# yflyzhang/RankPO

Hardware: AMD Instinct MI355X
Metric: query-passage pairs/sec (higher is better)
Workload: dtype bf16

## Files before the change

### include/rankpo_hip.h

```cpp
#ifndef RANKPO_HIP_H
#define RANKPO_HIP_H

#include <stddef.h>
#include <stdint.h>

#ifdef __cplusplus
extern "C" {
#endif

typedef void* rpo_stream_t;

typedef enum {
    RPO_OK = 0,
    RPO_ERR_INVALID_ARG = -1,
    RPO_ERR_UNSUPPORTED = -2,
    RPO_ERR_WORKSPACE = -3,
    RPO_ERR_LAUNCH = -4
} rpo_status;

typedef enum { RPO_DT_F32 = 0, RPO_DT_BF16 = 1, RPO_DT_F16 = 2 } rpo_dtype;
typedef enum { RPO_POOL_LAST = 0, RPO_POOL_CLS = 1 } rpo_pool_mode;
typedef enum { RPO_TARGET_INBATCH = 0, RPO_TARGET_FIRST = 1 } rpo_target_mode;
typedef enum { RPO_LOSS_SIGMOID = 0, RPO_LOSS_HINGE = 1 } rpo_loss_type;

// ... 86 lines not shown
                          int dtype, float lr, float beta1, float beta2, float eps, float weight_decay, const void* ls_state,
                          rpo_stream_t stream);

int rpo_swiglu_fwd(const void* g, const void* u, void* out, int64_t rows, int64_t cols, int64_t ld_gu, int64_t ld_out,
                   int dtype, rpo_stream_t stream);
int rpo_swiglu_bwd(const void* g, const void* u, const void* dout, void* dg, void* du, void* prod_out, int64_t rows,
                   int64_t cols, int64_t ld_gu, int64_t ld_dout, int64_t ld_dgu, int64_t ld_prod, int dtype,
                   rpo_stream_t stream);
int rpo_swiglu_bwd_t(const void* g, const void* u, const void* dout, void* dg, void* du, void* prod_t_out, void* dgu_t_out,
                     int64_t rows, int64_t cols, int64_t ld_gu, int64_t ld_dout, int64_t ld_dgu, int64_t ld_t, int dtype,
                     rpo_stream_t stream);
int rpo_rope(const void* x_in, void* x_out, int64_t row_stride, const float* cos_tab, const float* sin_tab,
             int64_t rows, int64_t heads, int64_t head_dim, int64_t period, int dtype, int backward,
             rpo_stream_t stream);

int rpo_transpose(const void* in, void* out, int64_t rows, int64_t cols, int64_t ld_in, int64_t ld_out, int dtype,
                  rpo_stream_t stream);

int rpo_add_rmsnorm_waves(int64_t rows);
int rpo_add_rmsnorm_fwd(const void* x, const void* delta, const void* weight, float eps, void* x_out, void* y_out,
                        float* rstd_out, int64_t rows, int64_t d, int dtype, rpo_stream_t stream);
int rpo_add_rmsnorm_bwd(const void* dy, const void* x_new, const void* weight, const float* rstd, const void* dres,
                        void* dx_out, float* dw_partial, int64_t rows, int64_t d, int dtype, rpo_stream_t stream);

int rpo_flash_attn_fwd(const void* q, const void* k, const void* v, int64_t q_stride, int64_t k_stride,
                       int64_t v_stride, const int* cu_seqlens, const int* tiles, int64_t ntiles, int64_t tile_cols,
                       int64_t total_tokens,
                       int64_t num_heads, int64_t num_kv_heads, int64_t head_dim, float scale, void* out,
                       int64_t out_stride, float* lse, int64_t lse_max_len, const float* rope_cos, const float* rope_sin,
                       int64_t rope_period, int64_t q_block, rpo_stream_t stream);

int rpo_flash_attn_bwd(const void* q, const void* k, const void* v, const void* out, const void* dout, int64_t q_stride,
                       int64_t k_stride, int64_t v_stride, int64_t out_stride, int64_t dout_stride,
                       const int* cu_seqlens, const int* q_tiles, int64_t n_q_tiles, int64_t q_tile_cols, const int* k_tiles,
                       int64_t n_k_tiles, int64_t key_block, int64_t sweep_down, int64_t total_tokens, int64_t num_heads,
                       int64_t num_kv_heads, int64_t head_dim, float scale, const float* lse, float* delta, void* dq, void* dk, void* dv,
                       int64_t dq_stride, int64_t dk_stride, int64_t dv_stride, const float* rope_cos, const float* rope_sin,
                       int64_t rope_period, int64_t q_block, rpo_stream_t stream);

int rpo_lastq_attn_fwd(const void* q, int64_t q_stride, const void* k, const void* v, int64_t k_stride, int64_t v_stride,
                       const int* cu_seqlens, int64_t num_seqs, int64_t num_heads, int64_t num_kv_heads, int64_t head_dim,
                       float scale, void* out, int64_t out_stride, float* lse, rpo_stream_t stream);
int rpo_lastq_attn_bwd(const void* q, int64_t q_stride, const void* k, const void* v, int64_t k_stride, int64_t v_stride,
                       const int* cu_seqlens, int64_t num_seqs, int64_t num_heads, int64_t num_kv_heads, int64_t head_dim,
                       float scale, const void* out, int64_t out_stride, const void* dout, int64_t dout_stride, const float* lse,
                       void* dq, int64_t dq_stride, void* dk, void* dv, int64_t dk_stride, int64_t dv_stride, rpo_stream_t stream);
// ... 104 lines not shown
```

### rankpo_amd/_lib.py

```python
from __future__ import annotations

import ctypes as C
import os

_HERE = os.path.dirname(os.path.abspath(__file__))
LIB_PATH = os.path.join(_HERE, "csrc", "librankpo_hip.so")

RPO_OK = 0
RPO_DT_F32, RPO_DT_BF16, RPO_DT_F16 = 0, 1, 2
RPO_POOL_LAST, RPO_POOL_CLS = 0, 1
(RPO_LS_SCALE, RPO_LS_MULT, RPO_LS_NORM, RPO_LS_SKIP, RPO_LS_GOOD_STEPS, RPO_LS_CUR_HYSTERESIS, RPO_LS_APPLIED_STEPS,
 RPO_LS_SKIPPED_STEPS, RPO_LS_FLOOR_HITS) = range(9)
RPO_LS_WORDS = 16
RPO_TARGET_INBATCH, RPO_TARGET_FIRST = 0, 1
RPO_LOSS_SIGMOID, RPO_LOSS_HINGE = 0, 1
RPO_BUILD_ONEWAVE64 = 1
RPO_NUM_METRICS = 9
METRIC_KEYS = (
    "rankpo_loss", "sft_loss", "rewards/chosen", "rewards/rejected", "rewards/accuracies",
    "rewards/margins", "scores/chosen", "scores/rejected", "scores/margins",
)


class RankPOParams(C.Structure):
# ... 27 lines not shown
    "rpo_rankpo_fwd": (C.c_int, [_vp, _vp, _vp, _vp, _i64, _i64, _i32, C.POINTER(RankPOParams), _vp, _vp, _vp, _vp, _vp, _vp]),
    "rpo_rankpo_bwd": (C.c_int, [_vp, _vp, _vp, _vp, _i64, _i64, _i32, _vp, _vp, _vp]),
    "rpo_adamw_step": (C.c_int, [_vp, _vp, _vp, _vp, _vp, _i64, _i32, _f32, _f32, _f32, _f32, _f32, _f32, _f32, _vp, _vp]),
    "rpo_sumsq_partial": (C.c_int, [_vp, _i64, _i32, _vp, _i32, _vp]),
    "rpo_loss_scale_update": (C.c_int, [_vp, _vp, _f32, _f32, _i32, _i32, _i32, _i32, _f32, _vp]),
    "rpo_adamw_step_scaled": (C.c_int, [_vp, _vp, _vp, _vp, _vp, _i64, _i32, _f32, _f32, _f32, _f32, _f32, _vp, _vp]),
    "rpo_swiglu_fwd": (C.c_int, [_vp, _vp, _vp, _i64, _i64, _i64, _i64, _i32, _vp]),
    "rpo_topk_merge": (C.c_int, [_vp, _i64, _i64, _i64, _i64, _i32, _i32, _vp, _vp, _i32, _vp]),
    "rpo_topk_merge_split": (C.c_int, [_vp, _i64, _i64, _i64, _i64, _i32, _i32, _i32, _vp, _vp, _i32, _vp]),
    "rpo_sim_topk_filter_ok": (C.c_int, [_i64, _i64, _i64]),
    "rpo_sim_topk_filter": (C.c_int, [_vp, _vp, _i64, _i64, _i64, _i32, _i64, _i32, _i32, _vp, _vp, _vp, _vp, _vp, _i32, _vp]),
    "rpo_sim_scores_f32": (C.c_int, [_vp, _vp, _i64, _i64, _i64, _i32, _vp, _i64, _vp]),
    "rpo_topk_merge_candidates": (C.c_int, [_vp, _vp, _vp, _i64, _i32, _i32, _vp, _vp, _vp, _vp]),
    "rpo_split_bf16x3": (C.c_int, [_vp, _i64, _i64, _i64, _vp, _i64, _vp, _vp]),
    "rpo_sim_planes_ok": (C.c_int, [_i64, _i64, _i64]),
    "rpo_sim_scores_f32_planes": (C.c_int, [_vp, _vp, _i64, _i64, _i64, _vp, _i64, _vp]),
    "rpo_sim_topk_filter_planes": (C.c_int, [_vp, _vp, _i64, _i64, _i64, _i64, _i32, _vp, _vp, _vp, _vp, _vp, _i32, _vp]),
    "rpo_swiglu_bwd": (C.c_int, [_vp, _vp, _vp, _vp, _vp, _vp, _i64, _i64, _i64, _i64, _i64, _i64, _i32, _vp]),
    "rpo_swiglu_bwd_t": (C.c_int, [_vp, _vp, _vp, _vp, _vp, _vp, _vp, _i64, _i64, _i64, _i64, _i64, _i64, _i32, _vp]),
    "rpo_transpose": (C.c_int, [_vp, _vp, _i64, _i64, _i64, _i64, _i32, _vp]),
    "rpo_add_rmsnorm_waves": (C.c_int, [_i64]),
    "rpo_add_rmsnorm_fwd": (C.c_int, [_vp, _vp, _vp, _f32, _vp, _vp, _vp, _i64, _i64, _i32, _vp]),
    "rpo_add_rmsnorm_bwd": (C.c_int, [_vp, _vp, _vp, _vp, _vp, _vp, _vp, _i64, _i64, _i32, _vp]),
    "rpo_flash_attn_fwd": (C.c_int, [_vp, _vp, _vp, _i64, _i64, _i64, _vp, _vp, _i64, _i64, _i64, _i64, _i64, _i64, _f32, _vp,
                                     _i64, _vp, _i64, _vp, _vp, _i64, _i64, _vp]),
    "rpo_flash_attn_bwd": (C.c_int, [_vp] * 5 + [_i64] * 5 + [_vp, _vp, _i64, _i64, _vp, _i64, _i64, _i64, _i64, _i64, _i64, _i64, _f32, _vp, _vp,
                                     _vp, _vp, _vp, _i64, _i64, _i64, _vp, _vp, _i64, _i64, _vp]),
    "rpo_lastq_attn_fwd": (C.c_int, [_vp, _i64, _vp, _vp, _i64, _i64, _vp, _i64, _i64, _i64, _i64, _f32, _vp, _i64, _vp, _vp]),
    "rpo_lastq_attn_bwd": (C.c_int, [_vp, _i64, _vp, _vp, _i64, _i64, _vp, _i64, _i64, _i64, _i64, _f32, _vp, _i64, _vp, _i64, _vp,
                                     _vp, _i64, _vp, _vp, _i64, _i64, _vp]),
    "rpo_rope": (C.c_int, [_vp, _vp, _i64, _vp, _vp, _i64, _i64, _i64, _i64, _i32, _i32, _vp]),
    "rpo_bidir_attn_fwd": (C.c_int, [_vp, _vp, _vp, _i64, _i64, _i64, _vp, _vp, _vp, _i64, _i64, _i64, _i64, _i64, _i64, _i64, _i32,
                                     _f32, _vp, _i64, _vp, _vp]),
    "rpo_add_layernorm_fwd": (C.c_int, [_vp, _i64, _vp, _i64, _vp, _vp, _f32, _vp, _i64, _i64, _i64, _i32, _vp]),
    "rpo_gelu_fwd": (C.c_int, [_vp, _i64, _i64, _i64, _i32, _vp]),
    "rpo_bert_embed_ln_fwd": (C.c_int, [_vp, _vp, _vp, _i64, _vp, _i64, _vp, _i64, _vp, _i64, _vp, _vp, _f32, _vp, _i64, _i64, _i32,
                                        _vp]),
    "rpo_bidir_attn_fwd_f32": (C.c_int, [_vp, _vp, _vp, _i64, _i64, _i64, _vp, _vp, _vp, _i64, _i64, _i64, _i64, _i64, _i64, _i64,
                                         _f32, _vp, _i64, _vp, _vp]),
    "rpo_add_layernorm_fwd_f32": (C.c_int, [_vp, _i64, _vp, _i64, _vp, _vp, _f32, _vp, _i64, _i64, _i64, _vp]),
    "rpo_gelu_fwd_f32": (C.c_int, [_vp, _i64, _i64, _i64, _vp]),
    "rpo_bert_embed_ln_fwd_f32": (C.c_int, [_vp, _vp, _vp, _i64, _vp, _i64, _vp, _i64, _vp, _i64, _vp, _vp, _f32, _vp, _i64, _i64,
                                            _vp]),
    "rpo_bidir_attn_train_fwd": (C.c_int, [_vp, _vp, _vp, _i64, _i64, _i64, _vp, _vp, _vp, _i64, _i64, _i64, _i64, _i64, _i64, _i64,
                                           _i32, _f32, _f32, _u64, _vp, _i64, _vp, _vp]),
    "rpo_bidir_attn_bwd": (C.c_int, [_vp, _vp, _vp, _i64, _i64, _i64, _vp, _i64, _vp, _i64, _vp, _vp, _vp, _vp, _i64, _vp, _i64,
# ... 55 lines not shown
```

### rankpo_amd/csrc/encoder_ops.hip

```cpp
#include "common.hpp"

namespace {

constexpr int kEwThreads = 256;

__device__ __forceinline__ float sigmoid_f(float x) { return 1.0f / (1.0f + __expf(-x)); }

template <typename T>
__global__ __launch_bounds__(kEwThreads) void swiglu_fwd_kernel(const T* __restrict__ g, const T* __restrict__ u,
                                                                T* __restrict__ out, int64_t rows, int vec_per_row,
                                                                int64_t ld_gu, int64_t ld_out) {
    constexpr int V = Elem<T>::kVec;
    const int64_t i = (int64_t)blockIdx.x * kEwThreads + threadIdx.x;
    const int64_t r = i / vec_per_row;
    if (r >= rows) return;
    const int c = (int)(i - r * vec_per_row) * V;
    Vec16<T> a, b, o;
    a.load_nt(g + r * ld_gu + c);
    b.load_nt(u + r * ld_gu + c);
#pragma unroll
    for (int k = 0; k < V; ++k) o.v[k] = a.v[k] * sigmoid_f(a.v[k]) * b.v[k];
    o.store_nt(out + r * ld_out + c);
}

// ... 551 lines not shown
        (delta && (!rpo_aligned16(delta) || !rpo_aligned16(x_out))))
        return RPO_ERR_UNSUPPORTED;
    hipStream_t st = (hipStream_t)stream;
    const int nw = norm_waves(rows, RPO_NORM_FWD_CAP);
    if (dtype == RPO_DT_BF16) return launch_norm_fwd<bf16_t>(x, delta, weight, eps, x_out, y_out, rstd_out, rows, d, nw, st);
    if (dtype == RPO_DT_F32) return launch_norm_fwd<float>(x, delta, weight, eps, x_out, y_out, rstd_out, rows, d, nw, st);
    return RPO_ERR_INVALID_ARG;
}

extern "C" int rpo_add_rmsnorm_bwd(const void* dy, const void* x_new, const void* weight, const float* rstd,
                                   const void* dres, void* dx_out, float* dw_partial, int64_t rows, int64_t d,
                                   int dtype, rpo_stream_t stream) {
    if (!dy || !x_new || !weight || !rstd || !dx_out || !dw_partial || rows <= 0 || d <= 0) return RPO_ERR_INVALID_ARG;
    const int V = dtype == RPO_DT_BF16 ? 8 : 4;
    if (d % V != 0 || !rpo_aligned16(dy) || !rpo_aligned16(x_new) || !rpo_aligned16(dx_out) || !rpo_aligned16(weight) ||
        !rpo_aligned16(dw_partial) || (dres && !rpo_aligned16(dres)))
        return RPO_ERR_UNSUPPORTED;
    hipStream_t st = (hipStream_t)stream;
    const int nw = rpo_add_rmsnorm_waves(rows);
    if (dtype == RPO_DT_BF16) return launch_norm_bwd<bf16_t>(dy, x_new, weight, rstd, dres, dx_out, dw_partial, rows, d, nw, st);
    if (dtype == RPO_DT_F32) return launch_norm_bwd<float>(dy, x_new, weight, rstd, dres, dx_out, dw_partial, rows, d, nw, st);
    return RPO_ERR_INVALID_ARG;
}
```

### rankpo_amd/distributed.py

```python
from __future__ import annotations

from typing import List, Optional

import torch
import torch.distributed as dist


def _all_gather_into(out: torch.Tensor, x: torch.Tensor, async_op=False):
    if dist.get_backend() == "nccl":
        return dist.all_gather_into_tensor(out.view(-1), x.reshape(-1), async_op=async_op)
    if x.is_cuda:
        host = [torch.empty(x.shape, dtype=x.dtype) for _ in range(out.shape[0])]
        dist.all_gather(host, x.cpu())
        out.copy_(torch.stack(host).to(out.device))
        return None
    return dist.all_gather(list(out.unbind(0)), x, async_op=async_op)


def deal_balanced(costs, hands: int) -> List[List[int]]:
    n = len(costs)
    if hands <= 0 or n % hands:
        raise ValueError(f"cannot deal {n} items into {hands} equal hands")
    per = n // hands
    total = [0.0] * hands
# ... 113 lines not shown

    def wait(self) -> torch.Tensor:
        if self.work is not None:
            self.work.wait()
            self.work = None
        return self.out.view((-1,) + tuple(self.x.shape[1:]))


class FusedQPGather:

    def __init__(self, qp: torch.Tensor, num_queries: int):
        self.nq = int(num_queries)
        self._g = EmbeddingGather(qp)

    def wait(self):
        out = self._g.out
        self._g.wait()
        d = out.shape[-1]
        return out[:, :self.nq].reshape(-1, d), out[:, self.nq:].reshape(-1, d)


def gather_embeddings(q: torch.Tensor, p: torch.Tensor):
    return FusedQPGather(torch.cat([q.detach(), p.detach()], 0), q.shape[0]).wait()


class FlatGradAllReducer:

    def __init__(self, params: List[torch.nn.Parameter], bucket_mb: float = 512.0, world_size: Optional[int] = None,
                 force_collectives: bool = False, shard: bool = False, rank: Optional[int] = None):
        self.params = [p for p in params if p.requires_grad]
        self.world = world_size if world_size is not None else (dist.get_world_size() if dist.is_initialized() else 1)
        self.rank = rank if rank is not None else (dist.get_rank() if dist.is_initialized() else 0)
        self.shard = bool(shard)
        assert self.params, "no trainable parameters"
        dtype, device = self.params[0].dtype, self.params[0].device
        assert all(p.dtype == dtype and p.device == device for p in self.params), "one dtype/device per reducer"
        order = list(reversed(self.params))
        i = 0
        while i < len(order):
            tag = getattr(order[i], "_rpo_fuse_group", None)
            j = i + 1
            if tag is not None:
                while j < len(order) and getattr(order[j], "_rpo_fuse_group", (None,))[0] is tag[0]:
                    j += 1
                order[i:j] = sorted(order[i:j], key=lambda p: p._rpo_fuse_group[1])
            i = j
# ... 7 lines not shown
            offs.append(n)
            n += (p.numel() + 7) // 8 * 8
            idxs.append(i)
            if n - start >= per or i == len(order) - 1:
                n = start + (n - start + quantum - 1) // quantum * quantum
                self.buckets.append((start, n, idxs))
                start, idxs = n, []
        self.numel = n
        self.flat = torch.zeros(n, dtype=dtype, device=device)
        self.order, self.offsets = order, offs
        for p, o in zip(order, offs):
            p.grad = self.flat[o:o + p.numel()].view_as(p)
        self.shard_offsets, self.shard_numel, self.grad_shards = [], 0, None
        if self.shard:
            for s_, e_, _ in self.buckets:
                self.shard_offsets.append(self.shard_numel)
                self.shard_numel += (e_ - s_) // self.world
            self.grad_shards = torch.zeros(self.shard_numel, dtype=dtype, device=device)
        self._bucket_of = {}
        for b, (_, _, ids) in enumerate(self.buckets):
            for i in ids:
                self._bucket_of[i] = b
        self._pending = [0] * len(self.buckets)
        self._works = []
        self._armed = False
        self.late_buckets = 0
        self._reduce = self.world > 1 or (force_collectives and dist.is_initialized())
        if self._reduce:
            for i, p in enumerate(order):
                p.register_post_accumulate_grad_hook(self._make_hook(i))

    def _make_hook(self, i):
        def hook(param):
            o = self.offsets[i]
            view = self.flat[o:o + param.numel()].view_as(param)
            if param.grad is not None and param.grad.data_ptr() != view.data_ptr():
                view.copy_(param.grad)
                param.grad = view
            if not self._armed:
                return
            b = self._bucket_of[i]
            self._pending[b] -= 1
            if self._pending[b] == 0:
                self._works.append(self._reduce_bucket(b))
        return hook

    def shard_view(self, b: int) -> torch.Tensor:
        s, e, _ = self.buckets[b]
        o = self.shard_offsets[b]
        return self.grad_shards[o:o + (e - s) // self.world]

    def _reduce_bucket(self, b: int):
        s, e, _ = self.buckets[b]
        if not self.shard:
            return dist.all_reduce(self.flat[s:e], op=dist.ReduceOp.SUM, async_op=True)
        out = self.shard_view(b)
        if dist.get_backend() == "nccl":
            return dist.reduce_scatter_tensor(out, self.flat[s:e], op=dist.ReduceOp.SUM, async_op=True)
        n = (e - s) // self.world
        dist.all_reduce(self.flat[s:e], op=dist.ReduceOp.SUM)
        out.copy_(self.flat[s + self.rank * n:s + (self.rank + 1) * n])
        return None

    def arm(self):
        self._armed = self._reduce
        self._pending = [len(ids) for _, _, ids in self.buckets]
        self._works = []

    def finish(self):
        if self._armed:
            for b, left in enumerate(self._pending):
                if left > 0:
                    self._works.append(self._reduce_bucket(b))
                    self._pending[b] = 0
                    self.late_buckets += 1
        for w in self._works:
            if w is not None:
                w.wait()
        self._works = []
        self._armed = False
        return 1.0 / self.world

    def reset(self):
        self._armed = False
        self._pending = [0] * len(self.buckets)
        for w in self._works:
            try:
                w.wait()
            except Exception:
                pass
        self._works = []
        if self.flat.is_cuda:
            torch.cuda.synchronize(self.flat.device)
        self.zero_()

    def zero_(self):
        self.flat.zero_()
```

### rankpo_amd/encoder.py

```python
from __future__ import annotations

import functools
import json
import math
import os
from types import SimpleNamespace
from typing import Optional

import torch
import torch.nn.functional as F
from torch import nn
from torch.utils.checkpoint import checkpoint

from . import ops as _ops


class EncoderConfig(SimpleNamespace):

    def to_dict(self):
        return dict(self.__dict__)

    @classmethod
    def from_json_file(cls, path):
        with open(path) as f:
            return cls(**json.load(f))


def llama_config(**kw) -> EncoderConfig:
    d = dict(architectures=["LlamaModel"], model_type="llama", vocab_size=128256, hidden_size=2048,
             intermediate_size=8192, num_hidden_layers=16, num_attention_heads=32, num_key_value_heads=8,
             head_dim=None, rms_norm_eps=1e-5, rope_theta=500000.0, rope_scaling=None,
             max_position_embeddings=131072, pad_token_id=None, attention_bias=False, mlp_bias=False,
             initializer_range=0.02, hidden_act="silu", padding_side="right", attention_dropout=0.0)
    d.update(kw)
    rp = d.pop("rope_parameters", None)
    if rp:
        if "rope_theta" in rp:
# ... 155 lines not shown
        cu_q = torch.arange(N + 1, device=q.device, dtype=torch.int32)
        return torch.ops.aten._flash_attention_forward(q, k, v, cu_q, ctx.cu, 1, ctx.max_len, 0.0, False, False)[0]
    outs, o0 = [], 0
    for i, n in enumerate(ctx.lens):
        a = F.scaled_dot_product_attention(q[i:i + 1].transpose(0, 1)[None], k[o0:o0 + n].transpose(0, 1)[None],
                                           v[o0:o0 + n].transpose(0, 1)[None], enable_gqa=k.shape[1] != q.shape[1])
        outs.append(a[0].transpose(0, 1))
        o0 += n
    return torch.cat(outs, 0)



def tag_fuse_group(*weights):
    key = object()
    for i, w in enumerate(weights):
        w._rpo_fuse_group = (key, i)


class _FusedWeight(torch.autograd.Function):

    @staticmethod
    def forward(ctx, *ws):
        ctx.rows = [w.shape[0] for w in ws]
        w0 = ws[0]
        adjacent = all(w.is_contiguous() and w.dim() == 2 and w.shape[1] == w0.shape[1] and w.dtype == w0.dtype
                       for w in ws)
        if adjacent:
            es = w0.element_size()
            for a, b in zip(ws[:-1], ws[1:]):
                if (a.untyped_storage().data_ptr() != b.untyped_storage().data_ptr()
                        or a.data_ptr() + a.numel() * es != b.data_ptr()):
                    adjacent = False
                    break
        if adjacent:
            return w0.detach().as_strided((sum(ctx.rows), w0.shape[1]), (w0.shape[1], 1), w0.storage_offset())
        return torch.cat([w.detach() for w in ws], 0)

    @staticmethod
    def backward(ctx, g):
        return tuple(g.split(ctx.rows, 0))


def fused_weight(ws):
    return _FusedWeight.apply(*ws)


class LlamaAttention(nn.Module):
    def __init__(self, cfg):
        super().__init__()
        self.nh, self.nkv, self.hd = cfg.num_attention_heads, cfg.num_key_value_heads, cfg.head_dim
        b = bool(cfg.attention_bias)
        self.q_proj = nn.Linear(cfg.hidden_size, self.nh * self.hd, bias=b)
        self.k_proj = nn.Linear(cfg.hidden_size, self.nkv * self.hd, bias=b)
        self.v_proj = nn.Linear(cfg.hidden_size, self.nkv * self.hd, bias=b)
        self.o_proj = nn.Linear(self.nh * self.hd, cfg.hidden_size, bias=b)
        tag_fuse_group(self.q_proj.weight, self.k_proj.weight, self.v_proj.weight)

    def _fused(self, x, mods):
        w = fused_weight([m.weight for m in mods])
        b = torch.cat([m.bias for m in mods], 0) if mods[0].bias is not None else None
        return _ops.linear(x, w, b)

    def forward(self, x, rope, attn_mask):
        N, L, _ = x.shape
        nq, nk = self.nh * self.hd, self.nkv * self.hd
        qkv = self._fused(x, (self.q_proj, self.k_proj, self.v_proj))
        fused = _ops.fused_encoder_ops_ok(x, self.hd)
# ... 831 lines not shown
```

### rankpo_amd/ops.py

```python
from __future__ import annotations

import ctypes as C
import threading
from dataclasses import dataclass
from typing import NamedTuple

import torch

from . import _lib
from ._lib import (RPO_DT_BF16, RPO_DT_F16, RPO_DT_F32, RPO_LOSS_HINGE, RPO_LOSS_SIGMOID, RPO_NUM_METRICS, RPO_POOL_CLS,
                   RPO_POOL_LAST, RPO_TARGET_FIRST, RPO_TARGET_INBATCH, METRIC_KEYS, RankPOParams, check)

F_NORMALIZE_EPS = 1e-12


def _dt(t: torch.Tensor) -> int:
    if t.dtype == torch.float32:
        return RPO_DT_F32
    if t.dtype == torch.bfloat16:
        return RPO_DT_BF16
    if t.dtype == torch.float16:
        return RPO_DT_F16
    raise TypeError(f"rankpo_amd HIP kernels take float32, bfloat16 or float16 tensors, got {t.dtype}")

# ... 256 lines not shown
WGRAD_MIXED = True
SWIGLU_DGU_T = True
SWIGLU_DGU_T_DEFAULT_MAX_BYTES = 6 * 2 ** 30
SWIGLU_DGU_T_MAX_BYTES = SWIGLU_DGU_T_DEFAULT_MAX_BYTES
SWIGLU_PROD_T = True
WGRAD_SPLIT_T = 4


def transpose2d(x):
    _need_gpu(x)
    lib = _lib.load()
    if x.dim() != 2 or x.stride(1) != 1:
        raise ValueError("transpose2d: a 2-D tensor with contiguous rows")
    R, C_ = x.shape
    out = torch.empty((C_, R), dtype=x.dtype, device=x.device)
    with torch.cuda.device(x.device):
        check(lib.rpo_transpose(x.data_ptr(), out.data_ptr(), R, C_, x.stride(0), R, _dt(x), _stream(x)), "rpo_transpose")
    return out


WGRAD_DY_T_HITS = 0


def wgrad(dy2, x2, dy_t=None):
    n, k = dy2.shape[1], x2.shape[1]
    if dy_t is not None and tuple(dy_t.shape) == (n, dy2.shape[0]) and dy_t.dtype == dy2.dtype and x2.stride(1) == 1:
        global WGRAD_DY_T_HITS
        WGRAD_DY_T_HITS += 1
        return torch.nn.functional.linear(dy_t, transpose2d(x2))
    if WGRAD_MIXED and dy2.is_cuda and dy2.dtype == torch.bfloat16 and dy2.stride(1) == 1 and x2.stride(1) == 1:
        if n >= 2 * k:
            return dy2.t() @ transpose2d(x2).t()
        if k >= 2 * n:
            return transpose2d(dy2) @ x2
        T, S = dy2.shape[0], WGRAD_SPLIT_T
        if S > 1 and T >= 32768 and T % S == 0 and n * k <= 8 * 1024 * 1024 and dy2.is_contiguous() and x2.is_contiguous():
            if _bmm_f32_out_ok(dy2.device):
                part = torch.bmm(dy2.view(S, T // S, n).transpose(1, 2), x2.view(S, T // S, k), out_dtype=torch.float32)
                return part.sum(0).to(dy2.dtype)
    return dy2.t() @ x2


_BMM_F32_OUT = {}


def _bmm_f32_out_ok(device) -> bool:
    key = str(device)
    if key not in _BMM_F32_OUT:
        try:
            a = torch.ones(2, 8, 16, dtype=torch.bfloat16, device=device)
            r = torch.bmm(a.transpose(1, 2), a, out_dtype=torch.float32)
            _BMM_F32_OUT[key] = bool(r.dtype == torch.float32 and float(r[0, 0, 0]) == 8.0)
        except Exception:
            _BMM_F32_OUT[key] = False
    return _BMM_F32_OUT[key]


def _wt(w):
    return transpose2d(w) if w.is_cuda and w.dtype in (torch.bfloat16, torch.float16, torch.float32) and w.stride(1) == 1 else w.t().contiguous()


class _LinearTN(torch.autograd.Function):

    @staticmethod
    def forward(ctx, x, w):
        ctx.save_for_backward(x, w)
        return torch.nn.functional.linear(x, w)

    @staticmethod
    def backward(ctx, dy):
        x, w = ctx.saved_tensors
        dx = dw = None
        if ctx.needs_input_grad[0]:
            dx = torch.nn.functional.linear(dy, _wt(w))
        if ctx.needs_input_grad[1]:
            dy_t = None
            tag = getattr(dy, "_rpo_transposed", None)
            if tag is not None and tag[1] == dy._version and tag[2] == dy.data_ptr():
                dy_t = tag[0]
            dw = wgrad(dy.reshape(-1, dy.shape[-1]), x.reshape(-1, x.shape[-1]), dy_t)
        return dx, dw


def linear(x, w, bias=None):
    if (bias is None and x.is_cuda and torch.is_grad_enabled() and (x.requires_grad or w.requires_grad)
            and LINEAR_TN):
        return _LinearTN.apply(x, w)
    return torch.nn.functional.linear(x, w, bias)


class recomputing:
    _tls = threading.local()

    @staticmethod
    def active():
        return getattr(recomputing._tls, "depth", 0) > 0

    def __enter__(self):
        recomputing._tls.depth = getattr(recomputing._tls, "depth", 0) + 1
        return self

    def __exit__(self, *exc):
        recomputing._tls.depth -= 1
        return False


class _SwiGLUDown(torch.autograd.Function):

    @staticmethod
    def forward(ctx, gu, weight, last_in_block=False):
        lib = _lib.load()
        gu = gu.contiguous()
        ff = gu.shape[-1] // 2
        rows = gu.numel() // (2 * ff)
        ctx.save_for_backward(gu, weight)
        if SKIP_RECOMPUTED_OUTPUT and last_in_block and recomputing.active():
            out = torch.empty(gu.shape[:-1] + (weight.shape[0],), dtype=gu.dtype, device=gu.device)
            return out.fill_(float("nan")) if POISON_SKIPPED_OUTPUT else out
        prod = _swiglu_fwd(lib, gu, torch.empty(gu.shape[:-1] + (ff,), dtype=gu.dtype, device=gu.device), rows, ff)
        return torch.nn.functional.linear(prod, weight)

    @staticmethod
    def backward(ctx, dy):
        gu, weight = ctx.saved_tensors
        lib = _lib.load()
        dy = dy.contiguous()
        ff = gu.shape[-1] // 2
        rows = gu.numel() // (2 * ff)
        es = gu.element_size()
        if LINEAR_TN:
            dprod = torch.nn.functional.linear(dy, _wt(weight))
        else:
            dprod = dy @ weight
        dgu = torch.empty_like(gu)
        want_dw = ctx.needs_input_grad[1]
        dy2 = dy.reshape(-1, dy.shape[-1])
        n = dy2.shape[1]
        if (want_dw and SWIGLU_PROD_T and WGRAD_MIXED and gu.dtype == torch.bfloat16 and ff >= 2 * n and rows >= 4096
                and rows % 8 == 0):
            prod_t = torch.empty((ff, rows), dtype=gu.dtype, device=gu.device)
            dgu_t = None
            if SWIGLU_DGU_T and 2 * ff * rows * es <= SWIGLU_DGU_T_MAX_BYTES:
                dgu_t = torch.empty((2 * ff, rows), dtype=gu.dtype, device=gu.device)
            with torch.cuda.device(gu.device):
                check(lib.rpo_swiglu_bwd_t(gu.data_ptr(), gu.data_ptr() + ff * es, dprod.data_ptr(), dgu.data_ptr(),
                                           dgu.data_ptr() + ff * es, prod_t.data_ptr(), _p(dgu_t), rows, ff, 2 * ff, ff, 2 * ff,
                                           rows, _dt(gu), _stream(gu)), "rpo_swiglu_bwd_t")
            if dgu_t is not None:
                dgu._rpo_transposed = (dgu_t, dgu._version, dgu.data_ptr())
            del dprod, dgu_t
            return dgu, torch.nn.functional.linear(transpose2d(dy2), prod_t), None
        with torch.cuda.device(gu.device):
            check(lib.rpo_swiglu_bwd(gu.data_ptr(), gu.data_ptr() + ff * es, dprod.data_ptr(), dgu.data_ptr(),
                                     dgu.data_ptr() + ff * es, dprod.data_ptr() if want_dw else None, rows, ff, 2 * ff,
                                     ff, 2 * ff, ff, _dt(gu), _stream(gu)), "rpo_swiglu_bwd")
        dW = None
        if want_dw:
            prod = dprod
            dW = wgrad(dy2, prod.reshape(-1, ff))
        return dgu, dW, None


def swiglu_down(gu, weight, last_in_block: bool = False):
    return _SwiGLUDown.apply(gu, weight, bool(last_in_block))


def fused_encoder_ops_ok(x, head_dim=None) -> bool:
    if not x.is_cuda or x.dtype not in (torch.float32, torch.bfloat16):
        return False
    v = 8 if x.dtype == torch.bfloat16 else 4
    return head_dim is None or (head_dim % 2 == 0 and (head_dim // 2) % v == 0)


class _AddRMSNorm(torch.autograd.Function):

    @staticmethod
    def forward(ctx, x, delta, weight, eps):
        lib = _lib.load()
        x = x.contiguous()
        d = x.shape[-1]
        rows = x.numel() // d
        y = torch.empty_like(x)
        rstd = torch.empty((rows,), dtype=torch.float32, device=x.device)
        x_new = torch.empty_like(x) if delta is not None else x
        if delta is not None:
            delta = delta.contiguous()
        with torch.cuda.device(x.device):
            check(lib.rpo_add_rmsnorm_fwd(x.data_ptr(), _p(delta), weight.data_ptr(), eps, _p(x_new if delta is not None else None),
                                          y.data_ptr(), rstd.data_ptr(), rows, d, _dt(x), _stream(x)), "rpo_add_rmsnorm_fwd")
        ctx.save_for_backward(x_new, weight, rstd)
        ctx.has_delta = delta is not None
        if delta is None:
            return y
        return x_new, y

    @staticmethod
    def backward(ctx, *grads):
        x_new, weight, rstd = ctx.saved_tensors
        lib = _lib.load()
        if ctx.has_delta:
            dres, dy = grads
        else:
            dres, dy = None, grads[0]
        d = x_new.shape[-1]
        rows = x_new.numel() // d
        if dy is None:
            return dres, (dres if ctx.has_delta else None), None, None
        dy = dy.contiguous()
        dres = None if dres is None else dres.contiguous()
        dx = torch.empty_like(x_new)
        nw = lib.rpo_add_rmsnorm_waves(rows)
        dwp = torch.empty((nw, d), dtype=torch.float32, device=x_new.device)
        with torch.cuda.device(x_new.device):
            check(lib.rpo_add_rmsnorm_bwd(dy.data_ptr(), x_new.data_ptr(), weight.data_ptr(), rstd.data_ptr(), _p(dres),
                                          dx.data_ptr(), dwp.data_ptr(), rows, d, _dt(x_new), _stream(x_new)),
                  "rpo_add_rmsnorm_bwd")
        dw = dwp.sum(0).to(weight.dtype) if ctx.needs_input_grad[2] else None
        return dx, (dx if ctx.has_delta else None), dw, None


def add_rmsnorm(x, delta, weight, eps):
    if delta is None:
        return x, _AddRMSNorm.apply(x, None, weight, eps)
    return _AddRMSNorm.apply(x, delta, weight, eps)


def fused_norm_ok(x) -> bool:
    if not x.is_cuda or x.dtype not in (torch.float32, torch.bfloat16):
        return False
    v = 8 if x.dtype == torch.bfloat16 else 4
    d = x.shape[-1]
    return d % v == 0 and d // v <= 64 * 8


class _Rope(torch.autograd.Function):

    @staticmethod
    def forward(ctx, x, cos, sin, heads, head_dim, grad_inplace):
        lib = _lib.load()
        row_len = x.shape[-1]
        rows = x.numel() // row_len
# ... 1058 lines not shown
```

### rankpo_amd/train_step.py

```python
from __future__ import annotations

import json
import math
from dataclasses import dataclass
from typing import Callable, Dict, Iterable, Optional, Union

import torch
import torch.distributed as dist
from torch import nn

from . import _lib
from ._lib import (RPO_DT_BF16, RPO_DT_F16, RPO_DT_F32, RPO_LS_APPLIED_STEPS, RPO_LS_CUR_HYSTERESIS, RPO_LS_FLOOR_HITS,
                   RPO_LS_GOOD_STEPS, RPO_LS_NORM, RPO_LS_SCALE, RPO_LS_SKIPPED_STEPS, RPO_LS_WORDS, check)
from .distributed import FlatGradAllReducer


def cosine_with_warmup(step: int, total_steps: int, warmup_steps: int) -> float:
    if step < warmup_steps:
        return step / max(1, warmup_steps)
    prog = (step - warmup_steps) / max(1, total_steps - warmup_steps)
    return max(0.0, 0.5 * (1.0 + math.cos(math.pi * prog)))


@dataclass
# ... 150 lines not shown
                                                param.numel(), self.dt, lr, b1, b2, self.eps, self.weight_decay,
                                                self.ls_state.data_ptr(), torch.cuda.current_stream(param.device).cuda_stream),
                      "rpo_adamw_step_scaled")
            return
        with torch.cuda.device(param.device):
            check(lib.rpo_adamw_step(param.data_ptr(), None if master is None else master.data_ptr(), grad.data_ptr(),
                                     m.data_ptr(), v.data_ptr(), param.numel(), self.dt, lr, b1, b2, self.eps, self.weight_decay,
                                     bc1, bc2, scale.data_ptr(), torch.cuda.current_stream(param.device).cuda_stream),
                  "rpo_adamw_step")

    def _grad_sumsq(self) -> torch.Tensor:
        if self.partition:
            ss = self._sumsq(self.reducer.grad_shards).reshape(1).clone()
            dist.all_reduce(ss, op=dist.ReduceOp.SUM)
            return ss
        return self._sumsq(self.reducer.flat).reshape(1)

    def grad_norm(self, pre_scale: float) -> torch.Tensor:
        norm = self._grad_sumsq()[0].sqrt() * pre_scale
        return norm if self.scaler is None else norm / self.loss_scale

    def step(self, grad_scale: float = 1.0, lr_mult: float = 1.0):
        r = self.reducer
        self.t += 1
        lr = self.lr * lr_mult
        if self.scaler is not None:
            self._scale_update(self._grad_sumsq(), grad_scale)
            self.last_grad_norm = self.ls_state.view(torch.float32)[RPO_LS_NORM].clone()
            bc1 = bc2 = scale = None
        else:
            scale = torch.full((1,), grad_scale, dtype=torch.float32, device=r.flat.device)
            if self.max_grad_norm is not None:
                norm = self.grad_norm(grad_scale)
                self.last_grad_norm = norm
                scale = scale * torch.clamp(self.max_grad_norm / (norm + 1e-6), max=1.0)
            b1, b2 = self.betas
            bc1, bc2 = 1.0 - b1 ** self.t, 1.0 - b2 ** self.t
        if not self.partition:
            self._adamw(self.flat_param, self.master, r.flat, self.exp_avg, self.exp_avg_sq, lr, bc1, bc2, scale)
            r.zero_()
            return
        works = []
        for b, (s, e, _) in enumerate(r.buckets):
            o, n = r.shard_offsets[b], (e - s) // r.world
            own = self._param_shard(b)
            self._adamw(own, None if self.master is None else self.master[o:o + n], r.grad_shards[o:o + n],
# ... 18 lines not shown
        return None


class TrainStep:

    def __init__(self, params, loss_fn: Callable[[Dict], torch.Tensor], *, lr=1e-5, weight_decay=0.0,
                 max_grad_norm=1.0, gradient_accumulation_steps=1, total_steps=1000, warmup_ratio=0.1,
                 bucket_mb=512.0, force_collectives=False, partition_optimizer=False,
                 loss_scale: Union[None, float, str, LossScaleConfig] = None):
        self.opt = FlatAdamW(params, lr=lr, weight_decay=weight_decay, max_grad_norm=max_grad_norm,
                             bucket_mb=bucket_mb, force_collectives=force_collectives, partition=partition_optimizer,
                             loss_scale=loss_scale)
        self.loss_fn = loss_fn
        self.gas = gradient_accumulation_steps
        self.total_steps = total_steps
        self.warmup_steps = int(math.ceil(total_steps * warmup_ratio))
        self.global_step = 0
        self.world = dist.get_world_size() if dist.is_initialized() else 1
        self._in_optimizer = False

    def micro_step(self, batch, last: bool) -> torch.Tensor:
        if last:
            self.opt.reducer.arm()
        loss = self.loss_fn(batch)
        scale = self.opt.loss_scale
        if scale is None:
            loss.backward()
        else:
            (loss.float() * scale).backward()
        return loss.detach()

    def loss_scale_state(self) -> Dict:
        return self.opt.loss_scale_state()

    def state_dict(self) -> Dict:
        out = {"global_step": self.global_step, "attempted_steps": self.opt.t}
        if self.opt.scaler is not None:
            out["loss_scale"] = self.opt.loss_scale_state()
        return out

    def load_state_dict(self, state: Dict):
        self.global_step = int(state["global_step"])
        self.opt.t = int(state["attempted_steps"])
        if self.opt.scaler is not None:
            self.opt.load_loss_scale_state(state["loss_scale"])
        elif state.get("loss_scale") is not None:
            raise ValueError("the state holds a loss scale but the parameters are not float16")

    def abort_step(self):
        if self._in_optimizer:
            raise RuntimeError("TrainStep.abort_step: the step failed inside the optimizer update; its state may be half-updated and "
                               "the step cannot be retried")
# ... 21 lines not shown
```

Before: 53.42.

## Write weight gradients directly into flat gradient buffer slots

Adds a gradient-slot mechanism so linear, SwiGLU-down and RMSNorm backward passes write or accumulate weight gradients straight into the flat all-reduce buffer, using mm out=/addmm_ and new HIP kernels for split-K partial reduction and norm dw reduction. This is meant to remove the temporary dW allocations, the autograd accumulate copies, and the separate sum/cast kernels. Zeroing becomes lazy, tracked per-slot state, with bookkeeping and hooks that the reducer must keep consistent. It adds complexity and risks double counting or stale gradients under recomputation or shared weights.

```diff
diff --git a/include/rankpo_hip.h b/include/rankpo_hip.h
--- a/include/rankpo_hip.h
+++ b/include/rankpo_hip.h
@@ -132,6 +132,12 @@
                         float* rstd_out, int64_t rows, int64_t d, int dtype, rpo_stream_t stream);
 int rpo_add_rmsnorm_bwd(const void* dy, const void* x_new, const void* weight, const float* rstd, const void* dres,
                         void* dx_out, float* dw_partial, int64_t rows, int64_t d, int dtype, rpo_stream_t stream);
+int rpo_add_rmsnorm_bwd_dw(const void* dy, const void* x_new, const void* weight, const float* rstd, const void* dres,
+                           void* dx_out, float* dw_partial, void* dw_out, int accumulate, int64_t rows, int64_t d, int dtype,
+                           rpo_stream_t stream);
+
+int rpo_wgrad_finish(const float* partials, int64_t S, int64_t n, int64_t k, void* out, int dtype, int accumulate,
+                     rpo_stream_t stream);
 
 int rpo_flash_attn_fwd(const void* q, const void* k, const void* v, int64_t q_stride, int64_t k_stride,
                        int64_t v_stride, const int* cu_seqlens, const int* tiles, int64_t ntiles, int64_t tile_cols,
diff --git a/rankpo_amd/_lib.py b/rankpo_amd/_lib.py
--- a/rankpo_amd/_lib.py
+++ b/rankpo_amd/_lib.py
@@ -73,6 +73,8 @@
     "rpo_add_rmsnorm_waves": (C.c_int, [_i64]),
     "rpo_add_rmsnorm_fwd": (C.c_int, [_vp, _vp, _vp, _f32, _vp, _vp, _vp, _i64, _i64, _i32, _vp]),
     "rpo_add_rmsnorm_bwd": (C.c_int, [_vp, _vp, _vp, _vp, _vp, _vp, _vp, _i64, _i64, _i32, _vp]),
+    "rpo_add_rmsnorm_bwd_dw": (C.c_int, [_vp, _vp, _vp, _vp, _vp, _vp, _vp, _vp, _i32, _i64, _i64, _i32, _vp]),
+    "rpo_wgrad_finish": (C.c_int, [_vp, _i64, _i64, _i64, _vp, _i32, _i32, _vp]),
     "rpo_flash_attn_fwd": (C.c_int, [_vp, _vp, _vp, _i64, _i64, _i64, _vp, _vp, _i64, _i64, _i64, _i64, _i64, _i64, _f32, _vp,
                                      _i64, _vp, _i64, _vp, _vp, _i64, _i64, _vp]),
     "rpo_flash_attn_bwd": (C.c_int, [_vp] * 5 + [_i64] * 5 + [_vp, _vp, _i64, _i64, _vp, _i64, _i64, _i64, _i64, _i64, _i64, _i64, _f32, _vp, _vp,
diff --git a/rankpo_amd/csrc/encoder_ops.hip b/rankpo_amd/csrc/encoder_ops.hip
--- a/rankpo_amd/csrc/encoder_ops.hip
+++ b/rankpo_amd/csrc/encoder_ops.hip
@@ -597,3 +597,174 @@
     if (dtype == RPO_DT_F32) return launch_norm_bwd<float>(dy, x_new, weight, rstd, dres, dx_out, dw_partial, rows, d, nw, st);
     return RPO_ERR_INVALID_ARG;
 }
+
+namespace {
+
+constexpr int kFinishThreads = 256;
+
+template <typename T>
+__global__ __launch_bounds__(kFinishThreads) void wgrad_finish_kernel(const float* __restrict__ part, T* __restrict__ out,
+                                                                      int S, int64_t nk, int64_t nvec, int accumulate) {
+    constexpr int V = Elem<T>::kVec;
+    const int64_t i = (int64_t)blockIdx.x * kFinishThreads + threadIdx.x;
+    if (i < nvec) {
+        float acc[V];
+#pragma unroll
+        for (int e = 0; e < V; ++e) acc[e] = 0.f;
+        for (int s = 0; s < S; ++s) {
+            const float* p = part + (int64_t)s * nk + i * V;
+#pragma unroll
+            for (int h = 0; h < V / 4; ++h) {
+                Vec16<float> t;
+                t.load_nt(p + 4 * h);
+#pragma unroll
+                for (int e = 0; e < 4; ++e) acc[4 * h + e] += t.v[e];
+            }
+        }
+        Vec16<T> o;
+        if (accumulate) {
+            o.load(out + i * V);
+#pragma unroll
+            for (int e = 0; e < V; ++e) o.v[e] += acc[e];
+        } else {
+#pragma unroll
+            for (int e = 0; e < V; ++e) o.v[e] = acc[e];
+        }
+        o.store(out + i * V);
+        return;
+    }
+    const int64_t j = nvec * V + (i - nvec);
+    if (j < nk) {
+        float acc = 0.f;
+        for (int s = 0; s < S; ++s) acc += part[(int64_t)s * nk + j];
+        if (accumulate) acc += Elem<T>::ld(out + j);
+        Elem<T>::st(out + j, acc);
+    }
+}
+
+constexpr int kDwChunk = 16, kDwGroupChunks = 4, kDwGroupRows = kDwChunk * kDwGroupChunks, kDwThreads = 64 * kDwGroupChunks;
+
+__device__ __forceinline__ void dw_sum_rows(const float* p, int64_t stride, int n, float (&a)[4]) {
+    a[0] = a[1] = a[2] = a[3] = 0.f;
+    if (n == kDwChunk) {
+        Vec16<float> t[kDwChunk];
+#pragma unroll
+        for (int w = 0; w < kDwChunk; ++w) t[w].load_nt(p + w * stride);
+#pragma unroll
+        for (int w = 0; w < kDwChunk; ++w) {
+#pragma unroll
+            for (int e = 0; e < 4; ++e) a[e] += t[w].v[e];
+        }
+    } else {
+        for (int w = 0; w < n; ++w) {
+            Vec16<float> t;
+            t.load_nt(p + w * stride);
+#pragma unroll
+            for (int e = 0; e < 4; ++e) a[e] += t.v[e];
+        }
+    }
+}
+
+__global__ __launch_bounds__(kDwThreads) void norm_dw_level1_kernel(float* dwp, int nw, int d) {
+    __shared__ float sm[kDwGroupChunks][64][4];
+    const int lane = threadIdx.x & 63, wv = threadIdx.x >> 6;
+    const int cv = blockIdx.x * 64 + lane;
+    const bool col_ok = cv < d / 4;
+    const int g0 = blockIdx.y * kDwGroupRows, w0 = g0 + wv * kDwChunk;
+    float a[4] = {0.f, 0.f, 0.f, 0.f};
+    if (col_ok && w0 < nw) dw_sum_rows(dwp + (int64_t)w0 * d + cv * 4, d, nw - w0 < kDwChunk ? nw - w0 : kDwChunk, a);
+#pragma unroll
+    for (int e = 0; e < 4; ++e) sm[wv][lane][e] = a[e];
+    __syncthreads();
+    if (wv == 0 && col_ok) {
+        Vec16<float> o;
+#pragma unroll
+        for (int e = 0; e < 4; ++e) o.v[e] = 0.f;
+        for (int j = 0; j < kDwGroupChunks; ++j) {
+#pragma unroll
+            for (int e = 0; e < 4; ++e) o.v[e] += sm[j][lane][e];
+        }
+        o.store(dwp + (int64_t)g0 * d + cv * 4);
+    }
+}
+
+template <typename T>
+__global__ __launch_bounds__(kDwThreads) void norm_dw_level2_kernel(const float* __restrict__ dwp, T* __restrict__ dw, int nw,
+                                                                    int d, int accumulate) {
+    __shared__ float sm[kDwGroupChunks][64][4];
+    const int lane = threadIdx.x & 63, wv = threadIdx.x >> 6;
+    const int cv = blockIdx.x * 64 + lane;
+    const bool col_ok = cv < d / 4;
+    const int ng = (nw + kDwGroupRows - 1) / kDwGroupRows, nsg = (ng + kDwChunk - 1) / kDwChunk;
+    float tot[4] = {0.f, 0.f, 0.f, 0.f};
+    for (int s0 = 0; s0 < nsg; s0 += kDwGroupChunks) {
+        const int gfirst = (s0 + wv) * kDwChunk;
+        float a[4] = {0.f, 0.f, 0.f, 0.f};
+        if (col_ok && gfirst < ng)
+            dw_sum_rows(dwp + (int64_t)gfirst * kDwGroupRows * d + cv * 4, (int64_t)kDwGroupRows * d,
+                        ng - gfirst < kDwChunk ? ng - gfirst : kDwChunk, a);
+#pragma unroll
+        for (int e = 0; e < 4; ++e) sm[wv][lane][e] = a[e];
+        __syncthreads();
+        if (wv == 0) {
+            for (int j = 0; j < kDwGroupChunks; ++j) {
+#pragma unroll
+                for (int e = 0; e < 4; ++e) tot[e] += sm[j][lane][e];
+            }
+        }
+        __syncthreads();
+    }
+    if (wv == 0 && col_ok) {
+#pragma unroll
+        for (int e = 0; e < 4; ++e) {
+            T* o = dw + cv * 4 + e;
+            Elem<T>::st(o, accumulate ? Elem<T>::ld(o) + tot[e] : tot[e]);
+        }
+    }
+}
+
+template <typename T>
+int launch_wgrad_finish(const float* part, void* out, int64_t S, int64_t nk, int accumulate, hipStream_t st) {
+    constexpr int V = Elem<T>::kVec;
+    const bool vec = nk % 4 == 0 && rpo_aligned16(part) && rpo_aligned16(out);
+    const int64_t nvec = vec ? nk / V : 0, threads = nvec + (nk - nvec * V);
+    const int64_t blocks = rpo_cdiv(threads, kFinishThreads);
+    if (blocks > 0x7fffffff) return RPO_ERR_UNSUPPORTED;
+    RPO_LAUNCH((wgrad_finish_kernel<T>), dim3((unsigned)blocks), dim3(kFinishThreads), 0, st, part, (T*)out, (int)S, nk, nvec,
+               accumulate);
+    return rpo_launch_status();
+}
+
+template <typename T>
+int launch_norm_dw_finish(float* dwp, void* dw, int nw, int64_t d, int accumulate, hipStream_t st) {
+    const unsigned gx = (unsigned)rpo_cdiv(d / 4, 64), ng = (unsigned)rpo_cdiv(nw, kDwGroupRows);
+    RPO_LAUNCH(norm_dw_level1_kernel, dim3(gx, ng), dim3(kDwThreads), 0, st, dwp, nw, (int)d);
+    const int rc = rpo_launch_status();
+    if (rc != RPO_OK) return rc;
+    RPO_LAUNCH((norm_dw_level2_kernel<T>), dim3(gx), dim3(kDwThreads), 0, st, (const float*)dwp, (T*)dw, nw, (int)d, accumulate);
+    return rpo_launch_status();
+}
+
+}
+
+extern "C" int rpo_add_rmsnorm_bwd_dw(const void* dy, const void* x_new, const void* weight, const float* rstd,
+                                      const void* dres, void* dx_out, float* dw_partial, void* dw_out, int accumulate,
+                                      int64_t rows, int64_t d, int dtype, rpo_stream_t stream) {
+    const int rc = rpo_add_rmsnorm_bwd(dy, x_new, weight, rstd, dres, dx_out, dw_partial, rows, d, dtype, stream);
+    if (rc != RPO_OK || !dw_out) return rc;
+    hipStream_t st = (hipStream_t)stream;
+    const int nw = rpo_add_rmsnorm_waves(rows);
+    if (dtype == RPO_DT_BF16) return launch_norm_dw_finish<bf16_t>(dw_partial, dw_out, nw, d, accumulate != 0, st);
+    return launch_norm_dw_finish<float>(dw_partial, dw_out, nw, d, accumulate != 0, st);
+}
+
+extern "C" int rpo_wgrad_finish(const float* partials, int64_t S, int64_t n, int64_t k, void* out, int dtype, int accumulate,
+                                rpo_stream_t stream) {
+    if (!partials || !out || S <= 0 || S > 0x7fffffff || n <= 0 || k <= 0) return RPO_ERR_INVALID_ARG;
+    if (!rpo_dtype_ok(dtype)) return RPO_ERR_INVALID_ARG;
+    hipStream_t st = (hipStream_t)stream;
+    const int64_t nk = n * k;
+    if (dtype == RPO_DT_BF16) return launch_wgrad_finish<bf16_t>(partials, out, S, nk, accumulate != 0, st);
+    if (dtype == RPO_DT_F16) return launch_wgrad_finish<f16_t>(partials, out, S, nk, accumulate != 0, st);
+    return launch_wgrad_finish<float>(partials, out, S, nk, accumulate != 0, st);
+}
diff --git a/rankpo_amd/distributed.py b/rankpo_amd/distributed.py
--- a/rankpo_amd/distributed.py
+++ b/rankpo_amd/distributed.py
@@ -1,5 +1,7 @@
 from __future__ import annotations
 
+import contextlib
+import weakref
 from typing import List, Optional
 
 import torch
@@ -159,6 +161,101 @@
 
 def gather_embeddings(q: torch.Tensor, p: torch.Tensor):
     return FusedQPGather(torch.cat([q.detach(), p.detach()], 0), q.shape[0]).wait()
+
+
+SLOT_CLEAN, SLOT_STALE, SLOT_LIVE, SLOT_LIVE_AUTOGRAD = 0, 1, 2, 3
+
+
+class GradSlot:
+    __slots__ = ("view", "state", "_claim", "shared", "_ready", "_open")
+
+    def __init__(self, view, ready, is_open):
+        self.view, self.state, self._claim, self.shared, self._ready, self._open = view, SLOT_CLEAN, None, False, ready, is_open
+
+    @property
+    def fresh(self):
+        return self.state == SLOT_CLEAN or self.state == SLOT_STALE
+
+    mixed = False
+
+    @property
+    def claimed(self):
+        return self._claim is not None and self._claim() is not None
+
+    def release(self):
+        self._claim, self.shared = None, False
+
+    def take(self, owner):
+        if not self._open():
+            return None
+        if self.claimed:
+            self.shared = True
+            return None
+        self._claim, self.shared = weakref.ref(owner), False
+        return self
+
+    def wrote(self, written=True):
+        if self.fresh and written:
+            self.state = SLOT_LIVE
+        self._claim = None
+        if not self.shared:
+            self._ready()
+
+    def land(self, g):
+        self.view.copy_(g) if self.fresh else self.view.add_(g)
+
+
+class GradSlotRange:
+    __slots__ = ("slots", "view")
+
+    def __init__(self, slots, view):
+        self.slots, self.view = slots, view
+
+    @property
+    def fresh(self):
+        return all(s.fresh for s in self.slots)
+
+    @property
+    def mixed(self):
+        return not self.fresh and any(s.fresh for s in self.slots)
+
+    def take(self, owner):
+        if not all(s._open() for s in self.slots):
+            return None
+        if any(s.claimed for s in self.slots):
+            for s in self.slots:
+                s.shared = s.shared or s.claimed
+            return None
+        for s in self.slots:
+            s.take(owner)
+        return self
+
+    def wrote(self, written=True):
+        for s in self.slots:
+            s.wrote(written)
+
+    def land(self, g):
+        r0 = 0
+        for s in self.slots:
+            n = s.view.shape[0]
+            s.land(g[r0:r0 + n])
+            r0 += n
+
+
+def fused_grad_slot(ws):
+    slots = [getattr(w, "_rpo_grad_slot", None) for w in ws]
+    if any(s is None for s in slots):
+        return None
+    v0 = slots[0].view
+    es = v0.element_size()
+    for a, b in zip(slots[:-1], slots[1:]):
+        if (a.view.untyped_storage().data_ptr() != b.view.untyped_storage().data_ptr()
+                or a.view.data_ptr() + a.view.numel() * es != b.view.data_ptr() or not b.view.is_contiguous()):
+            return None
+    if not v0.is_contiguous():
+        return None
+    rows = sum(s.view.shape[0] for s in slots)
+    return GradSlotRange(slots, v0.as_strided((rows, v0.shape[1]), (v0.shape[1], 1), v0.storage_offset()))
 
 
 class FlatGradAllReducer:
@@ -212,6 +309,7 @@
             for i in ids:
                 self._bucket_of[i] = b
         self._pending = [0] * len(self.buckets)
+        self._counted = [False] * len(order)
         self._works = []
         self._armed = False
         self.late_buckets = 0
@@ -219,6 +317,52 @@
         if self._reduce:
             for i, p in enumerate(order):
                 p.register_post_accumulate_grad_hook(self._make_hook(i))
+        self.slots = []
+        self._landing = False
+        for i, p in enumerate(order):
+            s = GradSlot(p.grad, self._make_ready(i), self._is_landing)
+            self.slots.append(s)
+            p._rpo_grad_slot = s
+            p.register_hook(self._make_pre_hook(s))
+
+    def _is_landing(self):
+        return self._landing
+
+    @contextlib.contextmanager
+    def landing_gradients(self):
+        prev, self._landing = self._landing, True
+        try:
+            yield self
+        finally:
+            self._landing = prev
+
+    def _count(self, i):
+        if not self._armed or self._counted[i]:
+            return
+        self._counted[i] = True
+        b = self._bucket_of[i]
+        self._pending[b] -= 1
+        if self._pending[b] == 0:
+            self._works.append(self._reduce_bucket(b))
+
+    def _make_ready(self, i):
+        return lambda: self._count(i)
+
+    @staticmethod
+    def _make_pre_hook(s):
+        def pre(grad):
+            if grad is None:
+                return
+            if s.state == SLOT_STALE:
+                s.view.zero_()
+            s.state = SLOT_LIVE_AUTOGRAD
+        return pre
+
+    def settle(self):
+        for s in self.slots:
+            if s.state == SLOT_STALE:
+                s.view.zero_()
+                s.state = SLOT_CLEAN
 
     def _make_hook(self, i):
         def hook(param):
@@ -227,12 +371,7 @@
             if param.grad is not None and param.grad.data_ptr() != view.data_ptr():
                 view.copy_(param.grad)
                 param.grad = view
-            if not self._armed:
-                return
-            b = self._bucket_of[i]
-            self._pending[b] -= 1
-            if self._pending[b] == 0:
-                self._works.append(self._reduce_bucket(b))
+            self._count(i)
         return hook
 
     def shard_view(self, b: int) -> torch.Tensor:
@@ -255,9 +394,11 @@
     def arm(self):
         self._armed = self._reduce
         self._pending = [len(ids) for _, _, ids in self.buckets]
+        self._counted = [False] * len(self.order)
         self._works = []
 
     def finish(self):
+        self.settle()
         if self._armed:
             for b, left in enumerate(self._pending):
                 if left > 0:
@@ -282,7 +423,25 @@
         self._works = []
         if self.flat.is_cuda:
             torch.cuda.synchronize(self.flat.device)
-        self.zero_()
+        self.flat.zero_()
+        for s in self.slots:
+            s.state = SLOT_CLEAN
+            s.release()
 
     def zero_(self):
-        self.flat.zero_()
+        run0 = None
+        for i, s in enumerate(self.slots):
+            s.release()
+            if s.state == SLOT_LIVE:
+                s.state = SLOT_STALE
+                if run0 is not None:
+                    self.flat[run0:self.offsets[i]].zero_()
+                    run0 = None
+                continue
+            if s.state == SLOT_STALE:
+                s.view.zero_()
+            s.state = SLOT_CLEAN
+            if run0 is None:
+                run0 = self.offsets[i]
+        if run0 is not None:
+            self.flat[run0:].zero_()
diff --git a/rankpo_amd/encoder.py b/rankpo_amd/encoder.py
--- a/rankpo_amd/encoder.py
+++ b/rankpo_amd/encoder.py
@@ -13,6 +13,7 @@
 from torch.utils.checkpoint import checkpoint
 
 from . import ops as _ops
+from .distributed import fused_grad_slot
 
 
 class EncoderConfig(SimpleNamespace):
@@ -214,6 +215,7 @@
     @staticmethod
     def forward(ctx, *ws):
         ctx.rows = [w.shape[0] for w in ws]
+        ctx.set_materialize_grads(False)
         w0 = ws[0]
         adjacent = all(w.is_contiguous() and w.dim() == 2 and w.shape[1] == w0.shape[1] and w.dtype == w0.dtype
                        for w in ws)
@@ -230,11 +232,18 @@
 
     @staticmethod
     def backward(ctx, g):
+        if g is None:
+            return (None,) * len(ctx.rows)
         return tuple(g.split(ctx.rows, 0))
 
 
 def fused_weight(ws):
-    return _FusedWeight.apply(*ws)
+    w = _FusedWeight.apply(*ws)
+    if _ops.GRAD_IN_PLACE and w.requires_grad and w.data_ptr() == ws[0].data_ptr():
+        slot = fused_grad_slot(ws)
+        if slot is not None:
+            w._rpo_grad_slot = slot
+    return w
 
 
 class LlamaAttention(nn.Module):
diff --git a/rankpo_amd/ops.py b/rankpo_amd/ops.py
--- a/rankpo_amd/ops.py
+++ b/rankpo_amd/ops.py
@@ -302,22 +302,67 @@
 WGRAD_DY_T_HITS = 0
 
 
-def wgrad(dy2, x2, dy_t=None):
+GRAD_IN_PLACE = True
+
+
+def take_grad_slot(w, ctx, needed=True):
+    if not (GRAD_IN_PLACE and needed) or recomputing.active():
+        return None
+    s = getattr(w, "_rpo_grad_slot", None)
+    return None if s is None else s.take(ctx)
+
+
+def _mm_into(slot, a, b):
+    if slot.mixed or slot.view.dtype != a.dtype:
+        slot.land(a @ b)
+    elif slot.fresh:
+        torch.mm(a, b, out=slot.view)
+    else:
+        slot.view.addmm_(a, b)
+    slot.wrote()
+
+
+def wgrad_finish(part, out, accumulate: bool):
+    _need_gpu(part, out)
+    if part.dtype != torch.float32 or not part.is_contiguous() or not out.is_contiguous() or tuple(out.shape) != tuple(part.shape[1:]):
+        raise ValueError("wgrad_finish: contiguous f32 [S, n, k] partials and a contiguous [n, k] output")
+    S, n, k = part.shape
+    with torch.cuda.device(part.device):
+        check(_lib.load().rpo_wgrad_finish(part.data_ptr(), S, n, k, out.data_ptr(), _dt(out), int(bool(accumulate)), _stream(part)),
+              "rpo_wgrad_finish")
+    return out
+
+
+def wgrad(dy2, x2, dy_t=None, slot=None):
     n, k = dy2.shape[1], x2.shape[1]
     if dy_t is not None and tuple(dy_t.shape) == (n, dy2.shape[0]) and dy_t.dtype == dy2.dtype and x2.stride(1) == 1:
         global WGRAD_DY_T_HITS
         WGRAD_DY_T_HITS += 1
+        if slot is not None:
+            return _mm_into(slot, dy_t, transpose2d(x2).t())
         return torch.nn.functional.linear(dy_t, transpose2d(x2))
     if WGRAD_MIXED and dy2.is_cuda and dy2.dtype == torch.bfloat16 and dy2.stride(1) == 1 and x2.stride(1) == 1:
         if n >= 2 * k:
+            if slot is not None:
+                return _mm_into(slot, dy2.t(), transpose2d(x2).t())
             return dy2.t() @ transpose2d(x2).t()
         if k >= 2 * n:
+            if slot is not None:
+                return _mm_into(slot, transpose2d(dy2), x2)
             return transpose2d(dy2) @ x2
         T, S = dy2.shape[0], WGRAD_SPLIT_T
         if S > 1 and T >= 32768 and T % S == 0 and n * k <= 8 * 1024 * 1024 and dy2.is_contiguous() and x2.is_contiguous():
             if _bmm_f32_out_ok(dy2.device):
                 part = torch.bmm(dy2.view(S, T // S, n).transpose(1, 2), x2.view(S, T // S, k), out_dtype=torch.float32)
-                return part.sum(0).to(dy2.dtype)
+                if slot is None:
+                    return part.sum(0).to(dy2.dtype)
+                if slot.mixed or slot.view.dtype != dy2.dtype:
+                    slot.land(part.sum(0).to(dy2.dtype))
+                else:
+                    wgrad_finish(part, slot.view, not slot.fresh)
+                return slot.wrote()
+    if slot is not None:
+        return _mm_into(slot, dy2.t(), x2)
     return dy2.t() @ x2
 
 
@@ -345,6 +390,7 @@
     @staticmethod
     def forward(ctx, x, w):
         ctx.save_for_backward(x, w)
+        ctx.slot = take_grad_slot(w, ctx, ctx.needs_input_grad[1])
         return torch.nn.functional.linear(x, w)
 
     @staticmethod
@@ -358,7 +404,7 @@
             tag = getattr(dy, "_rpo_transposed", None)
             if tag is not None and tag[1] == dy._version and tag[2] == dy.data_ptr():
                 dy_t = tag[0]
-            dw = wgrad(dy.reshape(-1, dy.shape[-1]), x.reshape(-1, x.shape[-1]), dy_t)
+            dw = wgrad(dy.reshape(-1, dy.shape[-1]), x.reshape(-1, x.shape[-1]), dy_t, ctx.slot)
         return dx, dw
 
 
@@ -394,6 +440,7 @@
         ff = gu.shape[-1] // 2
         rows = gu.numel() // (2 * ff)
         ctx.save_for_backward(gu, weight)
+        ctx.slot = take_grad_slot(weight, ctx, ctx.needs_input_grad[1])
         if SKIP_RECOMPUTED_OUTPUT and last_in_block and recomputing.active():
             out = torch.empty(gu.shape[:-1] + (weight.shape[0],), dtype=gu.dtype, device=gu.device)
             return out.fill_(float("nan")) if POISON_SKIPPED_OUTPUT else out
@@ -429,6 +476,8 @@
             if dgu_t is not None:
                 dgu._rpo_transposed = (dgu_t, dgu._version, dgu.data_ptr())
             del dprod, dgu_t
+            if ctx.slot is not None:
+                return dgu, _mm_into(ctx.slot, transpose2d(dy2), prod_t.t()), None
             return dgu, torch.nn.functional.linear(transpose2d(dy2), prod_t), None
         with torch.cuda.device(gu.device):
             check(lib.rpo_swiglu_bwd(gu.data_ptr(), gu.data_ptr() + ff * es, dprod.data_ptr(), dgu.data_ptr(),
@@ -437,7 +486,7 @@
         dW = None
         if want_dw:
             prod = dprod
-            dW = wgrad(dy2, prod.reshape(-1, ff))
+            dW = wgrad(dy2, prod.reshape(-1, ff), None, ctx.slot)
         return dgu, dW, None
 
 
@@ -470,6 +519,7 @@
                                           y.data_ptr(), rstd.data_ptr(), rows, d, _dt(x), _stream(x)), "rpo_add_rmsnorm_fwd")
         ctx.save_for_backward(x_new, weight, rstd)
         ctx.has_delta = delta is not None
+        ctx.slot = take_grad_slot(weight, ctx, ctx.needs_input_grad[2])
         if delta is None:
             return y
         return x_new, y
@@ -484,19 +534,37 @@
             dres, dy = None, grads[0]
         d = x_new.shape[-1]
         rows = x_new.numel() // d
+        slot = ctx.slot
         if dy is None:
+            if slot is not None:
+                slot.wrote(False)
             return dres, (dres if ctx.has_delta else None), None, None
         dy = dy.contiguous()
         dres = None if dres is None else dres.contiguous()
         dx = torch.empty_like(x_new)
         nw = lib.rpo_add_rmsnorm_waves(rows)
         dwp = torch.empty((nw, d), dtype=torch.float32, device=x_new.device)
+        if slot is not None and (slot.view.dtype != x_new.dtype or not slot.view.is_contiguous()):
+            slot.land(_AddRMSNorm._bwd(lib, dy, x_new, weight, rstd, dres, dx, dwp, rows, d).sum(0).to(weight.dtype))
+            slot.wrote()
+        elif slot is not None:
+            with torch.cuda.device(x_new.device):
+                check(lib.rpo_add_rmsnorm_bwd_dw(dy.data_ptr(), x_new.data_ptr(), weight.data_ptr(), rstd.data_ptr(), _p(dres),
+                                                 dx.data_ptr(), dwp.data_ptr(), slot.view.data_ptr(), int(not slot.fresh), rows, d,
+                                                 _dt(x_new), _stream(x_new)), "rpo_add_rmsnorm_bwd_dw")
+            slot.wrote()
+        else:
+            _AddRMSNorm._bwd(lib, dy, x_new, weight, rstd, dres, dx, dwp, rows, d)
+        dw = dwp.sum(0).to(weight.dtype) if ctx.needs_input_grad[2] and slot is None else None
+        return dx, (dx if ctx.has_delta else None), dw, None
+
+    @staticmethod
+    def _bwd(lib, dy, x_new, weight, rstd, dres, dx, dwp, rows, d):
         with torch.cuda.device(x_new.device):
             check(lib.rpo_add_rmsnorm_bwd(dy.data_ptr(), x_new.data_ptr(), weight.data_ptr(), rstd.data_ptr(), _p(dres),
                                           dx.data_ptr(), dwp.data_ptr(), rows, d, _dt(x_new), _stream(x_new)),
                   "rpo_add_rmsnorm_bwd")
-        dw = dwp.sum(0).to(weight.dtype) if ctx.needs_input_grad[2] else None
-        return dx, (dx if ctx.has_delta else None), dw, None
+        return dwp
 
 
 def add_rmsnorm(x, delta, weight, eps):
diff --git a/rankpo_amd/train_step.py b/rankpo_amd/train_step.py
--- a/rankpo_amd/train_step.py
+++ b/rankpo_amd/train_step.py
@@ -196,6 +196,7 @@
 
     def step(self, grad_scale: float = 1.0, lr_mult: float = 1.0):
         r = self.reducer
+        r.settle()
         self.t += 1
         lr = self.lr * lr_mult
         if self.scaler is not None:
@@ -260,12 +261,13 @@
     def micro_step(self, batch, last: bool) -> torch.Tensor:
         if last:
             self.opt.reducer.arm()
-        loss = self.loss_fn(batch)
-        scale = self.opt.loss_scale
-        if scale is None:
-            loss.backward()
-        else:
-            (loss.float() * scale).backward()
+        with self.opt.reducer.landing_gradients():
+            loss = self.loss_fn(batch)
+            scale = self.opt.loss_scale
+            if scale is None:
+                loss.backward()
+            else:
+                (loss.float() * scale).backward()
         return loss.detach()
 
     def loss_scale_state(self) -> Dict:
```

After: 53.56, median of 2. No clear change (+0.3%).
